# Dhia-naouali/dinov3-jax

Measured on NVIDIA H100. Metric: global_crops_per_sec, higher is better.
Workload: dtype bf16

## Files before the change

dinov3-jax_b200/csrc/gemm_tc.cu:

```cuda
#include <cstdlib>
#include <cstring>
#include "ptx.cuh"
#include "d3_internal.h"

namespace d3 {

constexpr int BM = 128;
constexpr int BK = 64;
constexpr int GEMM_THREADS = 384;

constexpr int EPI_RUNTIME = -1;
constexpr int EPI_FLAGS = EP_BIAS | EP_GELU | EP_STORE_PRE | EP_MUL_DGELU | EP_GAMMA | EP_RESID | EP_OUT_F32 | EP_ACCUM |
                          EP_SLABS;

template <int EF>
constexpr bool kStaged = EF != EPI_RUNTIME && (EF & (EP_SLABS | EP_ACCUM)) == 0;

template <int EF>
__device__ __forceinline__ bool epi_has(const GemmEpilogue& ep, int f) {
  return EF == EPI_RUNTIME ? (ep.flags & f) != 0 : (EF & f) != 0;
}

__device__ __forceinline__ float gelu_grad_epi(float u) {
  const float u2 = __fmul_rn(u, u);
// ... 15 lines not shown
  if (epi_has<EF>(ep, EP_ACCUM)) v = __fadd_rn(v, old);
  return v;
}

__device__ __forceinline__ float2 ld_pair(const float* p, bool vec, bool two) {
  if (vec) return *reinterpret_cast<const float2*>(p);
  return make_float2(p[0], two ? p[1] : 0.f);
}
__device__ __forceinline__ float2 ld_pair(const __nv_bfloat16* p, bool vec, bool two) {
  if (vec) return unpack_bf16(*reinterpret_cast<const uint32_t*>(p));
  return make_float2(__bfloat162float(p[0]), two ? __bfloat162float(p[1]) : 0.f);
}
__device__ __forceinline__ void st_pair(float* p, float a, float b, bool vec, bool two) {
  if (vec) {
    *reinterpret_cast<float2*>(p) = make_float2(a, b);
  } else {
    p[0] = a;
    if (two) p[1] = b;
  }
}
__device__ __forceinline__ void st_pair(__nv_bfloat16* p, float a, float b, bool vec, bool two) {
  if (vec) {
    *reinterpret_cast<uint32_t*>(p) = pack_bf16(a, b);
  } else {
    p[0] = __float2bfloat16(a);
    if (two) p[1] = __float2bfloat16(b);
  }
}

template <int BN>
__device__ __forceinline__ void epilogue_tile_runtime(const GemmEpilogue& ep, float (&acc)[2][BN / 2], int m0, int n0,
                                                      int M, int N, size_t slab_row0, int r_in, int c_in) {
  float* const out_f = reinterpret_cast<float*>(ep.out);
  __nv_bfloat16* const out_h = reinterpret_cast<__nv_bfloat16*>(ep.out);
  const bool aligned = (ep.flags & EP_SLOW) == 0;
#pragma unroll
  for (int mh = 0; mh < 2; ++mh)
#pragma unroll
    for (int h = 0; h < 2; ++h) {
      const size_t row = (size_t)(m0 + mh * 64 + r_in + 8 * h);
      if (row >= (size_t)M) continue;
      const size_t orow = slab_row0 + row;
#pragma unroll
      for (int i = 0; i < BN / 8; ++i) {
        const int n = n0 + 8 * i + c_in;
        if (n >= N) break;
        const bool two = n + 1 < N, vec = aligned && two;
        float2 b{}, u{}, g{}, x{}, o{};
        if (epi_has<EPI_RUNTIME>(ep, EP_BIAS)) b = ld_pair(ep.bias + n, vec, two);
        if (epi_has<EPI_RUNTIME>(ep, EP_MUL_DGELU)) u = ld_pair(ep.aux_in + row * ep.ld_aux + n, vec, two);
        if (epi_has<EPI_RUNTIME>(ep, EP_GAMMA)) g = ld_pair(ep.gamma + n, vec, two);
        if (epi_has<EPI_RUNTIME>(ep, EP_RESID)) x = ld_pair(ep.resid + row * ep.ld_resid + n, vec, two);
        if (epi_has<EPI_RUNTIME>(ep, EP_ACCUM)) o = ld_pair(out_f + orow * ep.ld_out + n, vec, two);
        float p0, p1;
        const float v0 = epi_value<EPI_RUNTIME>(ep, acc[mh][4 * i + 2 * h], b.x, u.x, g.x, x.x, o.x, p0);
        const float v1 = epi_value<EPI_RUNTIME>(ep, acc[mh][4 * i + 2 * h + 1], b.y, u.y, g.y, x.y, o.y, p1);
        if (epi_has<EPI_RUNTIME>(ep, EP_SCATTER)) {
          const unsigned long long g_idx = (unsigned long long)ep.sc_off + orow * ep.ld_out + n;
          const unsigned long long shard = (unsigned long long)ep.sc_shard;
          const unsigned r = (unsigned)(g_idx / shard);
          float* const dst = ep.sc_peer[r] + (g_idx - r * shard);
          if (!two) {
            atomicAdd(dst, v0);
          } else if (ep.sc_sys) {
            atomicAdd_system(dst, v0); atomicAdd_system(dst + 1, v1);
          } else {
            atomicAdd(reinterpret_cast<float2*>(dst), make_float2(v0, v1));
          }
          continue;
        }
        if (epi_has<EPI_RUNTIME>(ep, EP_STORE_PRE)) st_pair(ep.aux_out + row * ep.ld_aux + n, p0, p1, vec, two);
        if (epi_has<EPI_RUNTIME>(ep, EP_OUT_F32)) st_pair(out_f + orow * ep.ld_out + n, v0, v1, vec, two);
        else st_pair(out_h + orow * ep.ld_out + n, v0, v1, vec, two);
      }
    }
}

constexpr int STG_BOX = 64 * 128;
constexpr int STG_BYTES = 3 * STG_BOX;
__device__ __forceinline__ uint32_t sw128(int r, int byte) {
  return r * 128 + ((((byte >> 4) ^ r) & 7) << 4) + (byte & 15);
}

template <int BN, int EF>
__device__ __forceinline__ void epilogue_tile(const GemmEpilogue& ep, const CUtensorMap* tm_out,
                                              const CUtensorMap* tm_pre, float (&acc)[2][BN / 2], const float* s_bias,
                                              const float* s_gamma, uint8_t* stg, int& seq, int bar, int t, int m0,
                                              int n0, int M, int N, size_t slab_row0, int r_in, int c_in) {
  constexpr bool STAGED = kStaged<EF>;
  constexpr bool F32 = (EF & EP_OUT_F32) != 0;
  constexpr int OUT_BOXES = F32 ? 2 : 1;
  constexpr int CHUNK = (OUT_BOXES + ((EF & EP_STORE_PRE) ? 1 : 0)) * STG_BOX;
  constexpr int NBUF = STG_BYTES / CHUNK;
  static_assert(NBUF >= 1, "a chunk must fit the staging area");
  float* const out_f = reinterpret_cast<float*>(ep.out);
  __nv_bfloat16* const out_h = reinterpret_cast<__nv_bfloat16*>(ep.out);
#pragma unroll
  for (int mh = 0; mh < 2; ++mh)
#pragma unroll
    for (int cb = 0; cb < BN / 64; ++cb) {
      const int row0 = m0 + mh * 64, col0 = n0 + cb * 64;
      if (row0 >= M || col0 >= N) continue;
      float2 xr[2][8], xo[2][8];
      uint32_t xu[2][8];
#pragma unroll
      for (int h = 0; h < 2; ++h) {
        const size_t row = (size_t)row0 + r_in + 8 * h;
#pragma unroll
        for (int i = 0; i < 8; ++i) {
          const int n = col0 + 8 * i + c_in;
          if (row < (size_t)M && n < N) {
            if (epi_has<EF>(ep, EP_RESID))
              xr[h][i] = *reinterpret_cast<const float2*>(ep.resid + row * ep.ld_resid + n);
            if (epi_has<EF>(ep, EP_MUL_DGELU))
              xu[h][i] = *reinterpret_cast<const uint32_t*>(ep.aux_in + row * ep.ld_aux + n);
            if (epi_has<EF>(ep, EP_ACCUM))
              xo[h][i] = *reinterpret_cast<const float2*>(out_f + (slab_row0 + row) * ep.ld_out + n);
          }
        }
      }
      uint8_t* const buf = stg + (seq % NBUF) * CHUNK;
      if constexpr (STAGED) {
        if (t == 0) tma_store_wait_read<NBUF - 1>();
        named_bar_sync(bar, 128);
      }
#pragma unroll
      for (int h = 0; h < 2; ++h) {
        const int r = r_in + 8 * h;
        const size_t row = (size_t)row0 + r;
#pragma unroll
        for (int i = 0; i < 8; ++i) {
          const int cl = cb * 64 + 8 * i + c_in;
          const int n = n0 + cl;
          const float2 b = epi_has<EF>(ep, EP_BIAS) ? *reinterpret_cast<const float2*>(s_bias + cl) : float2{};
          const float2 g = epi_has<EF>(ep, EP_GAMMA) ? *reinterpret_cast<const float2*>(s_gamma + cl) : float2{};
          const float2 u = epi_has<EF>(ep, EP_MUL_DGELU) ? unpack_bf16(xu[h][i]) : float2{};
          float p0, p1;
          const float v0 = epi_value<EF>(ep, acc[mh][4 * (cl >> 3) + 2 * h], b.x, u.x, g.x, xr[h][i].x, xo[h][i].x, p0);
          const float v1 = epi_value<EF>(ep, acc[mh][4 * (cl >> 3) + 2 * h + 1], b.y, u.y, g.y, xr[h][i].y, xo[h][i].y,
                                         p1);
          if constexpr (STAGED) {
            if (epi_has<EF>(ep, EP_STORE_PRE))
              *reinterpret_cast<uint32_t*>(buf + OUT_BOXES * STG_BOX + sw128(r, 16 * i + 2 * c_in)) = pack_bf16(p0, p1);
            if constexpr (F32) {
              *reinterpret_cast<float2*>(buf + (i >> 2) * STG_BOX + sw128(r, 32 * (i & 3) + 4 * c_in)) =
                  make_float2(v0, v1);
            } else {
              *reinterpret_cast<uint32_t*>(buf + sw128(r, 16 * i + 2 * c_in)) = pack_bf16(v0, v1);
            }
          } else if (row < (size_t)M && n < N) {
            if (epi_has<EF>(ep, EP_STORE_PRE)) st_pair(ep.aux_out + row * ep.ld_aux + n, p0, p1, true, true);
            if constexpr (F32) st_pair(out_f + (slab_row0 + row) * ep.ld_out + n, v0, v1, true, true);
            else st_pair(out_h + (slab_row0 + row) * ep.ld_out + n, v0, v1, true, true);
          }
        }
      }
      if constexpr (STAGED) {
        fence_proxy_async_smem();
        named_bar_sync(bar, 128);
        if (t == 0) {
          tma_store_2d(tm_out, buf, col0, row0);
          if (F32 && col0 + 32 < N) tma_store_2d(tm_out, buf + STG_BOX, col0 + 32, row0);
          if constexpr ((EF & EP_STORE_PRE) != 0) tma_store_2d(tm_pre, buf + OUT_BOXES * STG_BOX, col0, row0);
          tma_store_commit();
        }
        ++seq;
      }
    }
}

template <int BN, bool STAGED>
struct Cfg {
  static constexpr int STAGES = (BN == 128 ? 6 : 8) - (STAGED ? 1 : 0);
  static constexpr int A_BYTES = BM * BK * 2;
  static constexpr int B_BYTES = BN * BK * 2;
  static constexpr int STAGE_BYTES = A_BYTES + B_BYTES;
  static constexpr int BAR_BYTES = 256;
  static constexpr int VEC_BYTES = 2 * 2 * BN * 4;
  static constexpr int VEC_END = STAGES * STAGE_BYTES + BAR_BYTES + VEC_BYTES;
  static constexpr int STG_OFF = (VEC_END + 1023) / 1024 * 1024;
  static constexpr int SMEM_BYTES = (STAGED ? STG_OFF + 2 * STG_BYTES : VEC_END) + 1024;
  static_assert(SMEM_BYTES <= 227 * 1024, "over the opt-in shared-memory limit");
};

struct WorkRange { int m0, n0, kb0, kb1; };
__device__ __forceinline__ WorkRange work_item(int w, int rank, int num_pairs, int num_k, int splits, int tile_n) {
  const int tile = w / splits, sp = w % splits;
  const int per = (num_k + splits - 1) / splits;
  WorkRange r;
  r.n0 = (2 * (tile % num_pairs) + rank) * tile_n;
  r.m0 = (tile / num_pairs) * BM;
  r.kb0 = sp * per;
  r.kb1 = min(num_k, r.kb0 + per);
  return r;
}

template <int BN, int A_MN, int B_MN>
__device__ __forceinline__ void mma_kblock(float (&acc)[2][BN / 2], uint32_t sa, uint32_t sb, bool first) {
  const uint64_t bd = B_MN ? gmma_desc_sw128(sb, 8192, 1024) : gmma_desc_sw128(sb, 16, 1024);
  constexpr uint64_t a_adv = A_MN ? (2048 >> 4) : (32 >> 4);
  constexpr uint64_t b_adv = B_MN ? (2048 >> 4) : (32 >> 4);
#pragma unroll
  for (int k = 0; k < BK / 16; ++k) {
    const uint32_t sc = (first && k == 0) ? 0u : 1u;
#pragma unroll
    for (int mh = 0; mh < 2; ++mh) {
      const uint64_t ad = A_MN ? gmma_desc_sw128(sa + mh * 8192, 8192, 1024) : gmma_desc_sw128(sa + mh * 8192, 16, 1024);
      if constexpr (BN == 128) wgmma_m64n128k16_ss<A_MN, B_MN>(acc[mh], ad + k * a_adv, bd + k * b_adv, sc);
      else wgmma_m64n64k16_ss<A_MN, B_MN>(acc[mh], ad + k * a_adv, bd + k * b_adv, sc);
    }
  }
}

template <int BN, int A_MN, int B_MN, int EF>
__global__ void __launch_bounds__(GEMM_THREADS, 1)
gemm_kernel(const __grid_constant__ CUtensorMap tmA, const __grid_constant__ CUtensorMap tmB,
            const __grid_constant__ CUtensorMap tmO, const __grid_constant__ CUtensorMap tmP, const GemmEpilogue ep,
            int M, int N, int K, int splits) {
  constexpr bool staged = kStaged<EF>;
  using C = Cfg<BN, staged>;
  static_assert(2 * C::STAGES * 8 <= C::BAR_BYTES, "mbarriers overflow their slot");
  extern __shared__ uint8_t smem_raw[];
  uint8_t* smem = reinterpret_cast<uint8_t*>((reinterpret_cast<uintptr_t>(smem_raw) + 1023) & ~uintptr_t(1023));
  uint64_t* full_bar = reinterpret_cast<uint64_t*>(smem + C::STAGES * C::STAGE_BYTES);
  uint64_t* empty_bar = full_bar + C::STAGES;
  float* vecs = reinterpret_cast<float*>(smem + C::STAGES * C::STAGE_BYTES + C::BAR_BYTES);

  const int wg = threadIdx.x >> 7;
  const int rank = blockIdx.x & 1;
  const int cluster = blockIdx.x >> 1, num_clusters = gridDim.x >> 1;
  if (threadIdx.x == 0) {
    tma_prefetch_desc(&tmA);
    tma_prefetch_desc(&tmB);
    if constexpr (staged) {
      tma_prefetch_desc(&tmO);
      if constexpr ((EF & EP_STORE_PRE) != 0) tma_prefetch_desc(&tmP);
    }
    for (int s = 0; s < C::STAGES; ++s) { mbar_init(&full_bar[s], 1); mbar_init(&empty_bar[s], 2); }
    fence_mbar_init();
  }
  cluster_sync();

  const int num_m = (M + BM - 1) / BM;
  const int num_pairs = ((N + BN - 1) / BN + 1) / 2;
  const int num_k = (K + BK - 1) / BK;
  const int num_work = num_m * num_pairs * splits;

  if (wg == 0) {
    setmaxnreg_dec<40>();
    if (threadIdx.x < 32 && elect_one()) {
      int stage = 0;
      uint32_t phase = 0;
      for (int w = cluster; w < num_work; w += num_clusters) {
        const WorkRange wr = work_item(w, rank, num_pairs, num_k, splits, BN);
        for (int kb = wr.kb0; kb < wr.kb1; ++kb) {
          mbar_wait(&empty_bar[stage], phase ^ 1);
          uint8_t* sa = smem + stage * C::STAGE_BYTES;
          uint8_t* sb = sa + C::A_BYTES;
          mbar_expect_tx(&full_bar[stage], C::STAGE_BYTES);
          if (A_MN) {
            tma_load_2d_multicast(&tmA, &full_bar[stage], sa + rank * 8192, wr.m0 + rank * 64, kb * BK, 0b11);
          } else {
            tma_load_2d_multicast(&tmA, &full_bar[stage], sa + rank * 8192, kb * BK, wr.m0 + rank * 64, 0b11);
          }
          if (B_MN) {
#pragma unroll
            for (int i = 0; i < BN / 64; ++i) tma_load_2d(&tmB, &full_bar[stage], sb + i * 8192, wr.n0 + i * 64, kb * BK);
          } else {
            tma_load_2d(&tmB, &full_bar[stage], sb, kb * BK, wr.n0);
          }
          if (++stage == C::STAGES) { stage = 0; phase ^= 1; }
        }
      }
    }
  } else {
    setmaxnreg_inc<232>();
    const int cw = wg - 1;
    const int t = threadIdx.x & 127;
    const int r_in = 16 * (t >> 5) + ((t & 31) >> 2);
    const int c_in = 2 * (t & 3);
    float* const s_bias = vecs + cw * 2 * BN;
    float* const s_gamma = s_bias + BN;
    constexpr bool stage_vecs = EF != EPI_RUNTIME && (EF & (EP_BIAS | EP_GAMMA)) != 0;
    uint8_t* const stg = smem + C::STG_OFF + cw * STG_BYTES;
    const uint32_t peer_empty = mapa_shared(smem_u32(empty_bar), rank ^ 1);
    int stg_seq = 0;
    int stage = 0;
    uint32_t phase = 0;
    int j = 0;
    for (int w = cluster; w < num_work; w += num_clusters, ++j) {
      const WorkRange wr = work_item(w, rank, num_pairs, num_k, splits, BN);
      const int nkb = wr.kb1 > wr.kb0 ? wr.kb1 - wr.kb0 : 0;
      if ((j & 1) != cw) {
        stage += nkb;
        phase ^= (stage / C::STAGES) & 1;
        stage %= C::STAGES;
        continue;
      }
      if constexpr (stage_vecs) {
        named_bar_sync(3 + cw, 128);
        if (t < BN && wr.n0 + t < N) {
          if constexpr ((EF & EP_BIAS) != 0) cp_async_4(s_bias + t, ep.bias + wr.n0 + t);
          if constexpr ((EF & EP_GAMMA) != 0) cp_async_4(s_gamma + t, ep.gamma + wr.n0 + t);
        }
      }
      if (j > 0) named_bar_sync(1 + cw, 256);
      float acc[2][BN / 2];
#pragma unroll
      for (int mh = 0; mh < 2; ++mh)
#pragma unroll
        for (int i = 0; i < BN / 2; ++i) acc[mh][i] = 0.f;
      int prev = -1;
      for (int kb = wr.kb0; kb < wr.kb1; ++kb) {
        mbar_wait(&full_bar[stage], phase);
        const uint32_t sa = smem_u32(smem + stage * C::STAGE_BYTES);
        fence_regs(acc[0]);
        fence_regs(acc[1]);
        wgmma_fence();
        mma_kblock<BN, A_MN, B_MN>(acc, sa, sa + C::A_BYTES, kb == wr.kb0);
        wgmma_commit();
        fence_regs(acc[0]);
        fence_regs(acc[1]);
        if (prev >= 0) {
          wgmma_wait<1>();
          if (t == 0) { mbar_arrive(&empty_bar[prev]); mbar_arrive_cluster(peer_empty + 8 * prev); }
        }
        prev = stage;
        if (++stage == C::STAGES) { stage = 0; phase ^= 1; }
      }
      if (w + num_clusters < num_work) named_bar_arrive(1 + (cw ^ 1), 256);
      wgmma_wait<0>();
      fence_regs(acc[0]);
      fence_regs(acc[1]);
      if (prev >= 0 && t == 0) { mbar_arrive(&empty_bar[prev]); mbar_arrive_cluster(peer_empty + 8 * prev); }
      if constexpr (stage_vecs) {
        cp_async_wait_all();
        named_bar_sync(3 + cw, 128);
      }
      if (nkb <= 0) continue;
      const size_t slab_row0 = epi_has<EF>(ep, EP_SLABS) ? (size_t)(w % splits) * M : 0;
      if constexpr (EF == EPI_RUNTIME) {
        epilogue_tile_runtime<BN>(ep, acc, wr.m0, wr.n0, M, N, slab_row0, r_in, c_in);
      } else {
        epilogue_tile<BN, EF>(ep, &tmO, &tmP, acc, s_bias, s_gamma, stg, stg_seq, 5 + cw, t, wr.m0, wr.n0, M, N,
                              slab_row0, r_in, c_in);
      }
    }
    if (staged && t == 0) tma_store_wait_all();
  }
  cluster_sync();
}

static int make_operand_map(CUtensorMap* map, const void* ptr, int mn, int k, int ld, int is_mn_major, int box_mn) {
  cuuint64_t dims[2], strides[1];
  cuuint32_t box[2], estr[2] = {1, 1};
  if (is_mn_major) {
    dims[0] = (cuuint64_t)mn; dims[1] = (cuuint64_t)k; box[0] = 64; box[1] = 64;
  } else {
    dims[0] = (cuuint64_t)k; dims[1] = (cuuint64_t)mn; box[0] = 64; box[1] = (cuuint32_t)box_mn;
  }
  strides[0] = (cuuint64_t)ld * 2;
  return encode_tensor_map_2d_bf16(map, ptr, dims, strides, box, estr);
}

template <int BN, int A_MN, int B_MN, int EF>
static int launch(const CUtensorMap& ta, const CUtensorMap& tb, const GemmEpilogue& ep, int M, int N, int K,
                  int splits, cudaStream_t stream) {
  using C = Cfg<BN, kStaged<EF>>;
  auto kern = gemm_kernel<BN, A_MN, B_MN, EF>;
  cudaLaunchAttribute attr{};
  attr.id = cudaLaunchAttributeClusterDimension;
  attr.val.clusterDim.x = 2;
  attr.val.clusterDim.y = 1;
  attr.val.clusterDim.z = 1;
  cudaLaunchConfig_t cfg{};
  cfg.blockDim = dim3(GEMM_THREADS);
  cfg.dynamicSmemBytes = C::SMEM_BYTES;
  cfg.stream = stream;
  cfg.attrs = &attr;
  cfg.numAttrs = 1;
  static int max_clusters = 0;
  if (max_clusters == 0) {
    cudaError_t e = cudaFuncSetAttribute(kern, cudaFuncAttributeMaxDynamicSharedMemorySize, C::SMEM_BYTES);
    if (e != cudaSuccess) return set_error(D3_ERR_CUDA, cudaGetErrorString(e));
    cfg.gridDim = dim3(2 * sm_count());
    e = cudaOccupancyMaxActiveClusters(&max_clusters, kern, &cfg);
    if (e != cudaSuccess) return set_error(D3_ERR_CUDA, cudaGetErrorString(e));
    if (max_clusters < 1) return set_error(D3_ERR_CUDA, "gemm: no 2-CTA cluster fits on the device");
  }
  CUtensorMap to{}, tp{};
  if constexpr (kStaged<EF>) {
    const int elt = (EF & EP_OUT_F32) ? 4 : 2;
    int rc = encode_tensor_map_2d(&to, ep.out, elt, N, M, (cuuint64_t)ep.ld_out * elt, 128 / elt, 64, 128);
    if (rc) return rc;
    if constexpr ((EF & EP_STORE_PRE) != 0) {
      rc = encode_tensor_map_2d(&tp, ep.aux_out, 2, N, M, (cuuint64_t)ep.ld_aux * 2, 64, 64, 128);
      if (rc) return rc;
    }
  }
  const int work = ((M + BM - 1) / BM) * (((N + BN - 1) / BN + 1) / 2) * splits;
  cfg.gridDim = dim3(2 * (work < max_clusters ? work : max_clusters));
  cudaError_t e = cudaLaunchKernelEx(&cfg, kern, ta, tb, to, tp, ep, M, N, K, splits);
  if (e == cudaSuccess) e = cudaPeekAtLastError();
  if (e != cudaSuccess) return set_error(D3_ERR_CUDA, cudaGetErrorString(e));
  count_launch();
  return D3_OK;
}

template <int BN>
static int dispatch(int a_mn, int b_mn, const CUtensorMap& ta, const CUtensorMap& tb, const GemmEpilogue& ep, int M,
                    int N, int K, int splits, cudaStream_t s) {
  if (!(ep.flags & (EP_SLOW | EP_SCATTER)) && N % 2 == 0) {
    const int f = ep.flags & EPI_FLAGS;
#define D3_EPI(A, B, F) \
    if (a_mn == A && b_mn == B && f == (F)) return launch<BN, A, B, (F)>(ta, tb, ep, M, N, K, splits, s);
    D3_EPI(0, 1, EP_BIAS)
    D3_EPI(0, 1, EP_BIAS | EP_OUT_F32)
    D3_EPI(0, 1, EP_BIAS | EP_GELU)
    D3_EPI(0, 1, EP_BIAS | EP_GELU | EP_STORE_PRE)
    D3_EPI(0, 1, EP_BIAS | EP_GAMMA | EP_RESID | EP_OUT_F32)
    D3_EPI(0, 1, EP_BIAS | EP_STORE_PRE | EP_GAMMA | EP_RESID | EP_OUT_F32)
    D3_EPI(0, 1, EP_BIAS | EP_GELU | EP_GAMMA | EP_RESID | EP_OUT_F32)
    D3_EPI(0, 1, EP_BIAS | EP_GELU | EP_STORE_PRE | EP_GAMMA | EP_RESID | EP_OUT_F32)
    D3_EPI(0, 1, EP_OUT_F32)
    D3_EPI(0, 0, 0)
    D3_EPI(0, 0, EP_MUL_DGELU)
    D3_EPI(0, 0, EP_OUT_F32)
    D3_EPI(1, 1, EP_OUT_F32 | EP_SLABS)
    D3_EPI(1, 1, EP_OUT_F32 | EP_ACCUM)
#undef D3_EPI
  }
  if (!a_mn && !b_mn) return launch<BN, 0, 0, EPI_RUNTIME>(ta, tb, ep, M, N, K, splits, s);
  if (!a_mn && b_mn) return launch<BN, 0, 1, EPI_RUNTIME>(ta, tb, ep, M, N, K, splits, s);
  if (a_mn && !b_mn) return launch<BN, 1, 0, EPI_RUNTIME>(ta, tb, ep, M, N, K, splits, s);
  return launch<BN, 1, 1, EPI_RUNTIME>(ta, tb, ep, M, N, K, splits, s);
}

int gemm_bf16(const void* A, int lda, int a_mn, const void* B, int ldb, int b_mn, int M, int N, int K,
              GemmEpilogue ep, int tile_n, int split_k, cudaStream_t stream) {
  if (M <= 0 || N <= 0 || K <= 0) return set_error(D3_ERR_ARG, "gemm: empty problem");
  if ((lda % 8) || (ldb % 8) || (reinterpret_cast<uintptr_t>(A) & 15) || (reinterpret_cast<uintptr_t>(B) & 15))
    return set_error(D3_ERR_ARG, "gemm: operands must be 16-byte aligned with ld % 8 == 0");
  const int sms = sm_count();
  const int num_k = (K + BK - 1) / BK;
  int bn = tile_n >= 256 ? 128 : tile_n;
  if (tile_n == 0) {
    const int cand[2] = {128, 64};
    long best = -1;
    for (int i = 0; i < 2; ++i) {
      const long tiles = (long)((M + BM - 1) / BM) * ((N + cand[i] - 1) / cand[i]);
      const long waves = (tiles + sms - 1) / sms;
      const long cost = waves * (cand[i] + 24);
      if (best < 0 || cost < best) { best = cost; bn = cand[i]; }
    }
  }
  const bool plain_f32 = (ep.flags & EP_OUT_F32) && !(ep.flags & (EP_BIAS | EP_GELU | EP_STORE_PRE | EP_MUL_DGELU |
                                                                  EP_GAMMA | EP_RESID));
  int splits = 1;
  if (split_k >= 1) {
    splits = split_k;
  } else if (plain_f32 && (ep.flags & EP_ACCUM)) {
    const long units = (long)((M + BM - 1) / BM) * ((N + bn - 1) / bn);
    if (units <= sms && num_k >= 16) {
      splits = units * 2 <= sms ? (int)(sms / units) : 1;
      if (splits < (num_k + 63) / 64) splits = (num_k + 63) / 64;
      if (splits > num_k / 4) splits = num_k / 4;
      if (splits < 1) splits = 1;
    }
  }
  if (ep.flags & EP_SCATTER) {
    if (!plain_f32) return set_error(D3_ERR_ARG, "gemm: SCATTER needs a plain fp32 output");
    if (ep.sc_world < 1 || ep.sc_world > 8 || ep.sc_shard <= 0 || (ep.sc_shard % 4) || (ep.sc_off % 4) || (ep.ld_out % 4))
      return set_error(D3_ERR_ARG, "gemm: SCATTER needs 1..8 ranks and 4-element aligned shard / offset / ld_out");
    if ((unsigned long long)ep.sc_off + (unsigned long long)(M - 1) * ep.ld_out + N > (unsigned long long)ep.sc_shard * ep.sc_world)
      return set_error(D3_ERR_ARG, "gemm: SCATTER output exceeds the sharded range");
  }
  if (splits > 1) {
    if (!plain_f32) return set_error(D3_ERR_ARG, "gemm: split-K needs a plain fp32 output");
    if (!(ep.flags & EP_ACCUM)) return set_error(D3_ERR_ARG, "gemm: split-K accumulates into out (set ACCUM, zero it first)");
    if (splits > num_k) splits = num_k;
  }
  if (ep.flags & EP_SCATTER) ep.flags &= ~EP_ACCUM;
  const int out_elt = (ep.flags & EP_OUT_F32) ? 4 : 2;
  bool aligned = ((uintptr_t)ep.out % 16 == 0) && ((ep.ld_out * out_elt) % 16 == 0);
  if (ep.flags & EP_BIAS) aligned = aligned && ((uintptr_t)ep.bias % 16 == 0);
  if (ep.flags & EP_GAMMA) aligned = aligned && ((uintptr_t)ep.gamma % 16 == 0);
  if (ep.flags & EP_RESID) aligned = aligned && ((uintptr_t)ep.resid % 16 == 0) && (ep.ld_resid % 4 == 0);
  if (ep.flags & EP_STORE_PRE) aligned = aligned && ((uintptr_t)ep.aux_out % 16 == 0) && (ep.ld_aux % 8 == 0);
  if (ep.flags & EP_MUL_DGELU) aligned = aligned && ((uintptr_t)ep.aux_in % 16 == 0) && (ep.ld_aux % 8 == 0);
  if (!aligned) ep.flags |= EP_SLOW;

  CUtensorMap ta, tb;
  int rc = make_operand_map(&ta, A, M, K, lda, a_mn, 64);
  if (rc) return rc;
  rc = make_operand_map(&tb, B, N, K, ldb, b_mn, bn);
  if (rc) return rc;
  float* ws = nullptr;
  GemmEpilogue out_ep = ep;
  if (splits > 1 && !(ep.flags & EP_SCATTER)) {
    ws = slab_workspace((size_t)splits * M * N, stream);
    if (!ws) return D3_ERR_CUDA;
    ep.out = ws;
    ep.ld_out = N;
    ep.flags = (ep.flags & ~(EP_ACCUM | EP_SLOW)) | EP_SLABS | (N % 4 ? EP_SLOW : 0);
  }
  switch (bn) {
    case 128: rc = dispatch<128>(a_mn, b_mn, ta, tb, ep, M, N, K, splits, stream); break;
    case 64: rc = dispatch<64>(a_mn, b_mn, ta, tb, ep, M, N, K, splits, stream); break;
    default: rc = set_error(D3_ERR_ARG, "gemm: bad tile N");
  }
  if (ws) {
    if (!rc) rc = slab_combine(ws, splits, (long long)M * N, M, N, reinterpret_cast<float*>(out_ep.out), out_ep.ld_out, stream);
    slab_release(ws, stream);
  }
  return rc;
}

}
```

dinov3-jax_b200/csrc/ptx.cuh:

```cuda
#pragma once
#include <cuda.h>
#include <cuda_runtime.h>
#include <cuda_bf16.h>
#include <stdint.h>

namespace d3 {

__device__ __forceinline__ uint32_t smem_u32(const void* p) {
  return static_cast<uint32_t>(__cvta_generic_to_shared(p));
}
__device__ __forceinline__ uint32_t lane_id() { return threadIdx.x & 31; }
__device__ __forceinline__ bool elect_one() {
  uint32_t pred;
  asm volatile("{\n\t.reg .pred p;\n\telect.sync _|p, 0xffffffff;\n\tselp.u32 %0, 1, 0, p;\n\t}" : "=r"(pred));
  return pred != 0;
}

__device__ __forceinline__ void mbar_init(uint64_t* bar, uint32_t count) {
  asm volatile("mbarrier.init.shared::cta.b64 [%0], %1;" ::"r"(smem_u32(bar)), "r"(count) : "memory");
}
__device__ __forceinline__ void fence_mbar_init() {
  asm volatile("fence.mbarrier_init.release.cluster;" ::: "memory");
}
__device__ __forceinline__ void mbar_expect_tx(uint64_t* bar, uint32_t bytes) {
// ... 39 lines not shown
  asm volatile("prefetch.tensormap [%0];" ::"l"(reinterpret_cast<uint64_t>(m)) : "memory");
}
__device__ __forceinline__ void tma_load_2d(const CUtensorMap* m, uint64_t* bar, void* dst, int c0, int c1) {
  asm volatile(
      "cp.async.bulk.tensor.2d.shared::cluster.global.mbarrier::complete_tx::bytes [%0], [%1, {%3, %4}], [%2];"
      ::"r"(smem_u32(dst)), "l"(reinterpret_cast<uint64_t>(m)), "r"(smem_u32(bar)), "r"(c0), "r"(c1)
      : "memory");
}
__device__ __forceinline__ void tma_load_2d_multicast(const CUtensorMap* m, uint64_t* bar, void* dst, int c0, int c1,
                                                      uint16_t cta_mask) {
  asm volatile(
      "cp.async.bulk.tensor.2d.shared::cluster.global.mbarrier::complete_tx::bytes.multicast::cluster"
      " [%0], [%1, {%3, %4}], [%2], %5;"
      ::"r"(smem_u32(dst)), "l"(reinterpret_cast<uint64_t>(m)), "r"(smem_u32(bar)), "r"(c0), "r"(c1), "h"(cta_mask)
      : "memory");
}

__device__ __forceinline__ uint32_t mapa_shared(uint32_t addr, uint32_t rank) {
  uint32_t r;
  asm volatile("mapa.shared::cluster.u32 %0, %1, %2;" : "=r"(r) : "r"(addr), "r"(rank));
  return r;
}
__device__ __forceinline__ void mbar_arrive_cluster(uint32_t cluster_addr) {
  asm volatile("mbarrier.arrive.shared::cluster.b64 _, [%0];" ::"r"(cluster_addr) : "memory");
}
__device__ __forceinline__ void cluster_sync() {
  asm volatile("barrier.cluster.arrive;\n\tbarrier.cluster.wait;" ::: "memory");
}

__device__ __forceinline__ void tma_store_2d(const CUtensorMap* m, const void* src, int c0, int c1) {
  asm volatile("cp.async.bulk.tensor.2d.global.shared::cta.bulk_group [%0, {%2, %3}], [%1];"
               ::"l"(reinterpret_cast<uint64_t>(m)), "r"(smem_u32(src)), "r"(c0), "r"(c1)
               : "memory");
}
__device__ __forceinline__ void tma_store_commit() { asm volatile("cp.async.bulk.commit_group;" ::: "memory"); }
template <int N>
__device__ __forceinline__ void tma_store_wait_read() { asm volatile("cp.async.bulk.wait_group.read %0;" ::"n"(N) : "memory"); }
__device__ __forceinline__ void tma_store_wait_all() { asm volatile("cp.async.bulk.wait_group 0;" ::: "memory"); }
__device__ __forceinline__ void tma_load_2d_cta(const CUtensorMap* m, uint64_t* bar, void* dst, int c0, int c1) {
  asm volatile(
      "cp.async.bulk.tensor.2d.shared::cta.global.mbarrier::complete_tx::bytes [%0], [%1, {%3, %4}], [%2];"
      ::"r"(smem_u32(dst)), "l"(reinterpret_cast<uint64_t>(m)), "r"(smem_u32(bar)), "r"(c0), "r"(c1)
      : "memory");
}

__device__ __forceinline__ uint64_t gmma_desc_sw128(uint32_t saddr, uint32_t lbo_bytes, uint32_t sbo_bytes) {
  uint64_t d = 0;
  d |= (uint64_t)((saddr >> 4) & 0x3FFF);
  d |= (uint64_t)((lbo_bytes >> 4) & 0x3FFF) << 16;
  d |= (uint64_t)((sbo_bytes >> 4) & 0x3FFF) << 32;
  d |= (uint64_t)1 << 62;
  return d;
}
__device__ __forceinline__ void wgmma_fence() { asm volatile("wgmma.fence.sync.aligned;" ::: "memory"); }
__device__ __forceinline__ void wgmma_commit() { asm volatile("wgmma.commit_group.sync.aligned;" ::: "memory"); }
template <int N>
__device__ __forceinline__ void wgmma_wait() { asm volatile("wgmma.wait_group.sync.aligned %0;" ::"n"(N) : "memory"); }
template <int R>
__device__ __forceinline__ void fence_regs(float (&d)[R]) {
#pragma unroll
  for (int i = 0; i < R; ++i) asm volatile("" : "+f"(d[i])::"memory");
}
template <int R>
__device__ __forceinline__ void setmaxnreg_inc() { asm volatile("setmaxnreg.inc.sync.aligned.u32 %0;" ::"n"(R)); }
template <int R>
__device__ __forceinline__ void setmaxnreg_dec() { asm volatile("setmaxnreg.dec.sync.aligned.u32 %0;" ::"n"(R)); }

template <int TA, int TB>
__device__ __forceinline__ void wgmma_m64n64k16_ss(float (&d)[32], uint64_t da, uint64_t db, uint32_t scale_d) {
  asm volatile(
      "{\n\t.reg .pred p;\n\tsetp.ne.b32 p, %34, 0;\n\t"
      "wgmma.mma_async.sync.aligned.m64n64k16.f32.bf16.bf16 {%0, %1, %2, %3, %4, %5, %6, %7, %8, %9, %10, %11, %12, %13, %14, %15, %16, %17, %18, %19, %20, %21, %22, %23, %24, %25, %26, %27, %28, %29, %30, %31}, %32, %33, p, 1, 1, %35, %36;\n\t}"
      : "+f"(d[0]), "+f"(d[1]), "+f"(d[2]), "+f"(d[3]), "+f"(d[4]), "+f"(d[5]), "+f"(d[6]), "+f"(d[7]), "+f"(d[8]), "+f"(d[9]), "+f"(d[10]), "+f"(d[11]), "+f"(d[12]), "+f"(d[13]), "+f"(d[14]), "+f"(d[15]), "+f"(d[16]), "+f"(d[17]), "+f"(d[18]), "+f"(d[19]), "+f"(d[20]), "+f"(d[21]), "+f"(d[22]), "+f"(d[23]), "+f"(d[24]), "+f"(d[25]), "+f"(d[26]), "+f"(d[27]), "+f"(d[28]), "+f"(d[29]), "+f"(d[30]), "+f"(d[31])
      : "l"(da), "l"(db), "r"(scale_d), "n"(TA), "n"(TB));
}
template <int TA, int TB>
__device__ __forceinline__ void wgmma_m64n128k16_ss(float (&d)[64], uint64_t da, uint64_t db, uint32_t scale_d) {
  asm volatile(
      "{\n\t.reg .pred p;\n\tsetp.ne.b32 p, %66, 0;\n\t"
      "wgmma.mma_async.sync.aligned.m64n128k16.f32.bf16.bf16 {%0, %1, %2, %3, %4, %5, %6, %7, %8, %9, %10, %11, %12, %13, %14, %15, %16, %17, %18, %19, %20, %21, %22, %23, %24, %25, %26, %27, %28, %29, %30, %31, %32, %33, %34, %35, %36, %37, %38, %39, %40, %41, %42, %43, %44, %45, %46, %47, %48, %49, %50, %51, %52, %53, %54, %55, %56, %57, %58, %59, %60, %61, %62, %63}, %64, %65, p, 1, 1, %67, %68;\n\t}"
      : "+f"(d[0]), "+f"(d[1]), "+f"(d[2]), "+f"(d[3]), "+f"(d[4]), "+f"(d[5]), "+f"(d[6]), "+f"(d[7]), "+f"(d[8]), "+f"(d[9]), "+f"(d[10]), "+f"(d[11]), "+f"(d[12]), "+f"(d[13]), "+f"(d[14]), "+f"(d[15]), "+f"(d[16]), "+f"(d[17]), "+f"(d[18]), "+f"(d[19]), "+f"(d[20]), "+f"(d[21]), "+f"(d[22]), "+f"(d[23]), "+f"(d[24]), "+f"(d[25]), "+f"(d[26]), "+f"(d[27]), "+f"(d[28]), "+f"(d[29]), "+f"(d[30]), "+f"(d[31]), "+f"(d[32]), "+f"(d[33]), "+f"(d[34]), "+f"(d[35]), "+f"(d[36]), "+f"(d[37]), "+f"(d[38]), "+f"(d[39]), "+f"(d[40]), "+f"(d[41]), "+f"(d[42]), "+f"(d[43]), "+f"(d[44]), "+f"(d[45]), "+f"(d[46]), "+f"(d[47]), "+f"(d[48]), "+f"(d[49]), "+f"(d[50]), "+f"(d[51]), "+f"(d[52]), "+f"(d[53]), "+f"(d[54]), "+f"(d[55]), "+f"(d[56]), "+f"(d[57]), "+f"(d[58]), "+f"(d[59]), "+f"(d[60]), "+f"(d[61]), "+f"(d[62]), "+f"(d[63])
      : "l"(da), "l"(db), "r"(scale_d), "n"(TA), "n"(TB));
}
template <int TB>
__device__ __forceinline__ void wgmma_m64n64k16_rs(float (&d)[32], const uint32_t (&a)[4], uint64_t db, uint32_t scale_d) {
  asm volatile(
      "{\n\t.reg .pred p;\n\tsetp.ne.b32 p, %37, 0;\n\t"
      "wgmma.mma_async.sync.aligned.m64n64k16.f32.bf16.bf16 {%0, %1, %2, %3, %4, %5, %6, %7, %8, %9, %10, %11, %12, %13, %14, %15, %16, %17, %18, %19, %20, %21, %22, %23, %24, %25, %26, %27, %28, %29, %30, %31}, {%32, %33, %34, %35}, %36, p, 1, 1, %38;\n\t}"
      : "+f"(d[0]), "+f"(d[1]), "+f"(d[2]), "+f"(d[3]), "+f"(d[4]), "+f"(d[5]), "+f"(d[6]), "+f"(d[7]), "+f"(d[8]), "+f"(d[9]), "+f"(d[10]), "+f"(d[11]), "+f"(d[12]), "+f"(d[13]), "+f"(d[14]), "+f"(d[15]), "+f"(d[16]), "+f"(d[17]), "+f"(d[18]), "+f"(d[19]), "+f"(d[20]), "+f"(d[21]), "+f"(d[22]), "+f"(d[23]), "+f"(d[24]), "+f"(d[25]), "+f"(d[26]), "+f"(d[27]), "+f"(d[28]), "+f"(d[29]), "+f"(d[30]), "+f"(d[31])
      : "r"(a[0]), "r"(a[1]), "r"(a[2]), "r"(a[3]), "l"(db), "r"(scale_d), "n"(TB));
}

__device__ __forceinline__ float ex2_approx(float x) {
  float y;
  asm("ex2.approx.ftz.f32 %0, %1;" : "=f"(y) : "f"(x));
  return y;
}
__device__ __forceinline__ float tanh_approx(float x) {
  float y;
  asm("tanh.approx.f32 %0, %1;" : "=f"(y) : "f"(x));
  return y;
}
__device__ __forceinline__ float gelu_tanh_fast(float u) {
  const float t = tanh_approx(u * (0.7978845608028654f + 0.0356774081363001f * u * u));
  const float h = 0.5f * u;
  return fmaf(h, t, h);
}
__device__ __forceinline__ float gelu_tanh_grad_fast(float u) {
  const float u2 = u * u;
  const float t = tanh_approx(u * (0.7978845608028654f + 0.0356774081363001f * u2));
  const float dz = 0.7978845608028654f + 0.1070322244089003f * u2;
  return 0.5f * (1.0f + t) + 0.5f * u * (1.0f - t * t) * dz;
}


__device__ __forceinline__ float gelu_tanh(float u) {
  float z = 0.7978845608028654f * (u + 0.044715f * u * u * u);
  float t = 1.0f - 2.0f / (__expf(2.0f * z) + 1.0f);
  return 0.5f * u * (1.0f + t);
}
__device__ __forceinline__ float gelu_tanh_grad(float u) {
  float u2 = u * u;
  float z = 0.7978845608028654f * (u + 0.044715f * u * u2);
  float t = 1.0f - 2.0f / (__expf(2.0f * z) + 1.0f);
  float dz = 0.7978845608028654f * (1.0f + 3.0f * 0.044715f * u2);
  return 0.5f * (1.0f + t) + 0.5f * u * (1.0f - t * t) * dz;
}
__device__ __forceinline__ uint32_t pack_bf16(float a, float b) {
  __nv_bfloat162 v = __floats2bfloat162_rn(a, b);
  return *reinterpret_cast<uint32_t*>(&v);
}
__device__ __forceinline__ float2 unpack_bf16(uint32_t u) {
  __nv_bfloat162 v = *reinterpret_cast<__nv_bfloat162*>(&u);
  return __bfloat1622float2(v);
}

}
```

Before: 370.4.

## Add 128x256 GEMM tile with cooperative consumer warpgroups and B multicast

Adds a BN=256 tile path in which both consumer warpgroups split one 128x256 tile, each issuing m64n256k16 wgmma on its own 64-row half. The cluster now pairs CTAs along M and multicasts the B operand, instead of pairing along N and multicasting A. When both operands are MN-major and no tile size is given, this wide tile is chosen by default. It aims to raise operand reuse and tensor-core efficiency per k-block, at the cost of fewer pipeline stages, higher register pressure from 128 fp32 accumulators per thread, and losing the ping-pong overlap of epilogue and MMA between warpgroups.

```diff
diff --git a/dinov3-jax_b200/csrc/gemm_tc.cu b/dinov3-jax_b200/csrc/gemm_tc.cu
--- a/dinov3-jax_b200/csrc/gemm_tc.cu
+++ b/dinov3-jax_b200/csrc/gemm_tc.cu
@@ -121,9 +121,9 @@
   return r * 128 + ((((byte >> 4) ^ r) & 7) << 4) + (byte & 15);
 }
 
-template <int BN, int EF>
+template <int MH, int BN, int EF>
 __device__ __forceinline__ void epilogue_tile(const GemmEpilogue& ep, const CUtensorMap* tm_out,
-                                              const CUtensorMap* tm_pre, float (&acc)[2][BN / 2], const float* s_bias,
+                                              const CUtensorMap* tm_pre, float (&acc)[MH][BN / 2], const float* s_bias,
                                               const float* s_gamma, uint8_t* stg, int& seq, int bar, int t, int m0,
                                               int n0, int M, int N, size_t slab_row0, int r_in, int c_in) {
   constexpr bool STAGED = kStaged<EF>;
@@ -135,7 +135,7 @@
   float* const out_f = reinterpret_cast<float*>(ep.out);
   __nv_bfloat16* const out_h = reinterpret_cast<__nv_bfloat16*>(ep.out);
 #pragma unroll
-  for (int mh = 0; mh < 2; ++mh)
+  for (int mh = 0; mh < MH; ++mh)
 #pragma unroll
     for (int cb = 0; cb < BN / 64; ++cb) {
       const int row0 = m0 + mh * 64, col0 = n0 + cb * 64;
@@ -210,32 +210,40 @@
 
 template <int BN, bool STAGED>
 struct Cfg {
-  static constexpr int STAGES = (BN == 128 ? 6 : 8) - (STAGED ? 1 : 0);
+  static constexpr bool WIDE = BN == 256;
+  static constexpr int STAGES = (BN == 256 ? 4 : BN == 128 ? 6 : 8) - (STAGED ? 1 : 0);
   static constexpr int A_BYTES = BM * BK * 2;
   static constexpr int B_BYTES = BN * BK * 2;
   static constexpr int STAGE_BYTES = A_BYTES + B_BYTES;
   static constexpr int BAR_BYTES = 256;
-  static constexpr int VEC_BYTES = 2 * 2 * BN * 4;
+  static constexpr int VEC_BYTES = (WIDE ? 1 : 2) * 2 * BN * 4;
   static constexpr int VEC_END = STAGES * STAGE_BYTES + BAR_BYTES + VEC_BYTES;
   static constexpr int STG_OFF = (VEC_END + 1023) / 1024 * 1024;
   static constexpr int SMEM_BYTES = (STAGED ? STG_OFF + 2 * STG_BYTES : VEC_END) + 1024;
   static_assert(SMEM_BYTES <= 227 * 1024, "over the opt-in shared-memory limit");
 };
 
-struct WorkRange { int m0, n0, kb0, kb1; };
-__device__ __forceinline__ WorkRange work_item(int w, int rank, int num_pairs, int num_k, int splits, int tile_n) {
-  const int tile = w / splits, sp = w % splits;
+struct WorkRange { int m0, n0, kb0, kb1, sp; };
+template <int BN>
+__device__ __forceinline__ WorkRange work_item(int w, int rank, int num_n, int num_tiles, int num_k, int splits) {
+  const int tile = w % num_tiles, sp = w / num_tiles;
   const int per = (num_k + splits - 1) / splits;
   WorkRange r;
-  r.n0 = (2 * (tile % num_pairs) + rank) * tile_n;
-  r.m0 = (tile / num_pairs) * BM;
+  if constexpr (BN == 256) {
+    r.n0 = (tile % num_n) * BN;
+    r.m0 = (2 * (tile / num_n) + rank) * BM;
+  } else {
+    r.n0 = (2 * (tile % num_n) + rank) * BN;
+    r.m0 = (tile / num_n) * BM;
+  }
   r.kb0 = sp * per;
   r.kb1 = min(num_k, r.kb0 + per);
+  r.sp = sp;
   return r;
 }
 
-template <int BN, int A_MN, int B_MN>
-__device__ __forceinline__ void mma_kblock(float (&acc)[2][BN / 2], uint32_t sa, uint32_t sb, bool first) {
+template <int MH, int BN, int A_MN, int B_MN>
+__device__ __forceinline__ void mma_kblock(float (&acc)[MH][BN / 2], uint32_t sa, uint32_t sb, bool first) {
   const uint64_t bd = B_MN ? gmma_desc_sw128(sb, 8192, 1024) : gmma_desc_sw128(sb, 16, 1024);
   constexpr uint64_t a_adv = A_MN ? (2048 >> 4) : (32 >> 4);
   constexpr uint64_t b_adv = B_MN ? (2048 >> 4) : (32 >> 4);
@@ -243,9 +251,10 @@
   for (int k = 0; k < BK / 16; ++k) {
     const uint32_t sc = (first && k == 0) ? 0u : 1u;
 #pragma unroll
-    for (int mh = 0; mh < 2; ++mh) {
+    for (int mh = 0; mh < MH; ++mh) {
       const uint64_t ad = A_MN ? gmma_desc_sw128(sa + mh * 8192, 8192, 1024) : gmma_desc_sw128(sa + mh * 8192, 16, 1024);
-      if constexpr (BN == 128) wgmma_m64n128k16_ss<A_MN, B_MN>(acc[mh], ad + k * a_adv, bd + k * b_adv, sc);
+      if constexpr (BN == 256) wgmma_m64n256k16_ss<A_MN, B_MN>(acc[mh], ad + k * a_adv, bd + k * b_adv, sc);
+      else if constexpr (BN == 128) wgmma_m64n128k16_ss<A_MN, B_MN>(acc[mh], ad + k * a_adv, bd + k * b_adv, sc);
       else wgmma_m64n64k16_ss<A_MN, B_MN>(acc[mh], ad + k * a_adv, bd + k * b_adv, sc);
     }
   }
@@ -258,6 +267,9 @@
             int M, int N, int K, int splits) {
   constexpr bool staged = kStaged<EF>;
   using C = Cfg<BN, staged>;
+  constexpr bool WIDE = C::WIDE;
+  constexpr int MH = WIDE ? 1 : 2;
+  static_assert(!WIDE || EF != EPI_RUNTIME, "run-time flags run on the 128-wide tile");
   static_assert(2 * C::STAGES * 8 <= C::BAR_BYTES, "mbarriers overflow their slot");
   extern __shared__ uint8_t smem_raw[];
   uint8_t* smem = reinterpret_cast<uint8_t*>((reinterpret_cast<uintptr_t>(smem_raw) + 1023) & ~uintptr_t(1023));
@@ -275,15 +287,16 @@
       tma_prefetch_desc(&tmO);
       if constexpr ((EF & EP_STORE_PRE) != 0) tma_prefetch_desc(&tmP);
     }
-    for (int s = 0; s < C::STAGES; ++s) { mbar_init(&full_bar[s], 1); mbar_init(&empty_bar[s], 2); }
+    for (int s = 0; s < C::STAGES; ++s) { mbar_init(&full_bar[s], 1); mbar_init(&empty_bar[s], WIDE ? 4 : 2); }
     fence_mbar_init();
   }
   cluster_sync();
 
   const int num_m = (M + BM - 1) / BM;
-  const int num_pairs = ((N + BN - 1) / BN + 1) / 2;
+  const int num_n = WIDE ? (N + BN - 1) / BN : ((N + BN - 1) / BN + 1) / 2;
   const int num_k = (K + BK - 1) / BK;
-  const int num_work = num_m * num_pairs * splits;
+  const int num_tiles = (WIDE ? (num_m + 1) / 2 : num_m) * num_n;
+  const int num_work = num_tiles * splits;
 
   if (wg == 0) {
     setmaxnreg_dec<40>();
@@ -291,22 +304,37 @@
       int stage = 0;
       uint32_t phase = 0;
       for (int w = cluster; w < num_work; w += num_clusters) {
-        const WorkRange wr = work_item(w, rank, num_pairs, num_k, splits, BN);
+        const WorkRange wr = work_item<BN>(w, rank, num_n, num_tiles, num_k, splits);
         for (int kb = wr.kb0; kb < wr.kb1; ++kb) {
           mbar_wait(&empty_bar[stage], phase ^ 1);
           uint8_t* sa = smem + stage * C::STAGE_BYTES;
           uint8_t* sb = sa + C::A_BYTES;
           mbar_expect_tx(&full_bar[stage], C::STAGE_BYTES);
-          if (A_MN) {
-            tma_load_2d_multicast(&tmA, &full_bar[stage], sa + rank * 8192, wr.m0 + rank * 64, kb * BK, 0b11);
+          if constexpr (WIDE) {
+#pragma unroll
+            for (int i = 0; i < 2; ++i) {
+              if (A_MN) tma_load_2d(&tmA, &full_bar[stage], sa + i * 8192, wr.m0 + i * 64, kb * BK);
+              else tma_load_2d(&tmA, &full_bar[stage], sa + i * 8192, kb * BK, wr.m0 + i * 64);
+            }
+            if (B_MN) {
+#pragma unroll
+              for (int i = 2 * rank; i < 2 * rank + 2; ++i)
+                tma_load_2d_multicast(&tmB, &full_bar[stage], sb + i * 8192, wr.n0 + i * 64, kb * BK, 0b11);
+            } else {
+              tma_load_2d_multicast(&tmB, &full_bar[stage], sb + rank * 16384, kb * BK, wr.n0 + rank * 128, 0b11);
+            }
           } else {
-            tma_load_2d_multicast(&tmA, &full_bar[stage], sa + rank * 8192, kb * BK, wr.m0 + rank * 64, 0b11);
-          }
-          if (B_MN) {
-#pragma unroll
-            for (int i = 0; i < BN / 64; ++i) tma_load_2d(&tmB, &full_bar[stage], sb + i * 8192, wr.n0 + i * 64, kb * BK);
-          } else {
-            tma_load_2d(&tmB, &full_bar[stage], sb, kb * BK, wr.n0);
+            if (A_MN) {
+              tma_load_2d_multicast(&tmA, &full_bar[stage], sa + rank * 8192, wr.m0 + rank * 64, kb * BK, 0b11);
+            } else {
+              tma_load_2d_multicast(&tmA, &full_bar[stage], sa + rank * 8192, kb * BK, wr.m0 + rank * 64, 0b11);
+            }
+            if (B_MN) {
+#pragma unroll
+              for (int i = 0; i < BN / 64; ++i) tma_load_2d(&tmB, &full_bar[stage], sb + i * 8192, wr.n0 + i * 64, kb * BK);
+            } else {
+              tma_load_2d(&tmB, &full_bar[stage], sb, kb * BK, wr.n0);
+            }
           }
           if (++stage == C::STAGES) { stage = 0; phase ^= 1; }
         }
@@ -318,9 +346,11 @@
     const int t = threadIdx.x & 127;
     const int r_in = 16 * (t >> 5) + ((t & 31) >> 2);
     const int c_in = 2 * (t & 3);
-    float* const s_bias = vecs + cw * 2 * BN;
+    float* const s_bias = vecs + (WIDE ? 0 : cw * 2 * BN);
     float* const s_gamma = s_bias + BN;
     constexpr bool stage_vecs = EF != EPI_RUNTIME && (EF & (EP_BIAS | EP_GAMMA)) != 0;
+    constexpr int VEC_THREADS = WIDE ? 256 : 128;
+    const int vt = WIDE ? threadIdx.x - 128 : t;
     uint8_t* const stg = smem + C::STG_OFF + cw * STG_BYTES;
     const uint32_t peer_empty = mapa_shared(smem_u32(empty_bar), rank ^ 1);
     int stg_seq = 0;
@@ -328,38 +358,38 @@
     uint32_t phase = 0;
     int j = 0;
     for (int w = cluster; w < num_work; w += num_clusters, ++j) {
-      const WorkRange wr = work_item(w, rank, num_pairs, num_k, splits, BN);
+      const WorkRange wr = work_item<BN>(w, rank, num_n, num_tiles, num_k, splits);
       const int nkb = wr.kb1 > wr.kb0 ? wr.kb1 - wr.kb0 : 0;
-      if ((j & 1) != cw) {
+      if (!WIDE && (j & 1) != cw) {
         stage += nkb;
         phase ^= (stage / C::STAGES) & 1;
         stage %= C::STAGES;
         continue;
       }
       if constexpr (stage_vecs) {
-        named_bar_sync(3 + cw, 128);
-        if (t < BN && wr.n0 + t < N) {
-          if constexpr ((EF & EP_BIAS) != 0) cp_async_4(s_bias + t, ep.bias + wr.n0 + t);
-          if constexpr ((EF & EP_GAMMA) != 0) cp_async_4(s_gamma + t, ep.gamma + wr.n0 + t);
-        }
-      }
-      if (j > 0) named_bar_sync(1 + cw, 256);
-      float acc[2][BN / 2];
-#pragma unroll
-      for (int mh = 0; mh < 2; ++mh)
+        named_bar_sync(3 + cw * !WIDE, VEC_THREADS);
+        if (vt < BN && wr.n0 + vt < N) {
+          if constexpr ((EF & EP_BIAS) != 0) cp_async_4(s_bias + vt, ep.bias + wr.n0 + vt);
+          if constexpr ((EF & EP_GAMMA) != 0) cp_async_4(s_gamma + vt, ep.gamma + wr.n0 + vt);
+        }
+      }
+      if (!WIDE && j > 0) named_bar_sync(1 + cw, 256);
+      float acc[MH][BN / 2];
+#pragma unroll
+      for (int mh = 0; mh < MH; ++mh)
 #pragma unroll
         for (int i = 0; i < BN / 2; ++i) acc[mh][i] = 0.f;
       int prev = -1;
       for (int kb = wr.kb0; kb < wr.kb1; ++kb) {
         mbar_wait(&full_bar[stage], phase);
         const uint32_t sa = smem_u32(smem + stage * C::STAGE_BYTES);
-        fence_regs(acc[0]);
-        fence_regs(acc[1]);
+#pragma unroll
+        for (int mh = 0; mh < MH; ++mh) fence_regs(acc[mh]);
         wgmma_fence();
-        mma_kblock<BN, A_MN, B_MN>(acc, sa, sa + C::A_BYTES, kb == wr.kb0);
+        mma_kblock<MH, BN, A_MN, B_MN>(acc, sa + (WIDE ? cw * 8192 : 0), sa + C::A_BYTES, kb == wr.kb0);
         wgmma_commit();
-        fence_regs(acc[0]);
-        fence_regs(acc[1]);
+#pragma unroll
+        for (int mh = 0; mh < MH; ++mh) fence_regs(acc[mh]);
         if (prev >= 0) {
           wgmma_wait<1>();
           if (t == 0) { mbar_arrive(&empty_bar[prev]); mbar_arrive_cluster(peer_empty + 8 * prev); }
@@ -367,22 +397,22 @@
         prev = stage;
         if (++stage == C::STAGES) { stage = 0; phase ^= 1; }
       }
-      if (w + num_clusters < num_work) named_bar_arrive(1 + (cw ^ 1), 256);
+      if (!WIDE && w + num_clusters < num_work) named_bar_arrive(1 + (cw ^ 1), 256);
       wgmma_wait<0>();
-      fence_regs(acc[0]);
-      fence_regs(acc[1]);
+#pragma unroll
+      for (int mh = 0; mh < MH; ++mh) fence_regs(acc[mh]);
       if (prev >= 0 && t == 0) { mbar_arrive(&empty_bar[prev]); mbar_arrive_cluster(peer_empty + 8 * prev); }
       if constexpr (stage_vecs) {
         cp_async_wait_all();
-        named_bar_sync(3 + cw, 128);
+        named_bar_sync(3 + cw * !WIDE, VEC_THREADS);
       }
       if (nkb <= 0) continue;
-      const size_t slab_row0 = epi_has<EF>(ep, EP_SLABS) ? (size_t)(w % splits) * M : 0;
+      const size_t slab_row0 = epi_has<EF>(ep, EP_SLABS) ? (size_t)wr.sp * M : 0;
       if constexpr (EF == EPI_RUNTIME) {
         epilogue_tile_runtime<BN>(ep, acc, wr.m0, wr.n0, M, N, slab_row0, r_in, c_in);
       } else {
-        epilogue_tile<BN, EF>(ep, &tmO, &tmP, acc, s_bias, s_gamma, stg, stg_seq, 5 + cw, t, wr.m0, wr.n0, M, N,
-                              slab_row0, r_in, c_in);
+        epilogue_tile<MH, BN, EF>(ep, &tmO, &tmP, acc, s_bias, s_gamma, stg, stg_seq, 5 + cw, t,
+                                  wr.m0 + (WIDE ? cw * 64 : 0), wr.n0, M, N, slab_row0, r_in, c_in);
       }
     }
     if (staged && t == 0) tma_store_wait_all();
@@ -437,7 +467,8 @@
       if (rc) return rc;
     }
   }
-  const int work = ((M + BM - 1) / BM) * (((N + BN - 1) / BN + 1) / 2) * splits;
+  const int num_m = (M + BM - 1) / BM, num_n = (N + BN - 1) / BN;
+  const int work = (BN == 256 ? (num_m + 1) / 2 * num_n : num_m * ((num_n + 1) / 2)) * splits;
   cfg.gridDim = dim3(2 * (work < max_clusters ? work : max_clusters));
   cudaError_t e = cudaLaunchKernelEx(&cfg, kern, ta, tb, to, tp, ep, M, N, K, splits);
   if (e == cudaSuccess) e = cudaPeekAtLastError();
@@ -469,10 +500,14 @@
     D3_EPI(1, 1, EP_OUT_F32 | EP_ACCUM)
 #undef D3_EPI
   }
-  if (!a_mn && !b_mn) return launch<BN, 0, 0, EPI_RUNTIME>(ta, tb, ep, M, N, K, splits, s);
-  if (!a_mn && b_mn) return launch<BN, 0, 1, EPI_RUNTIME>(ta, tb, ep, M, N, K, splits, s);
-  if (a_mn && !b_mn) return launch<BN, 1, 0, EPI_RUNTIME>(ta, tb, ep, M, N, K, splits, s);
-  return launch<BN, 1, 1, EPI_RUNTIME>(ta, tb, ep, M, N, K, splits, s);
+  if constexpr (BN == 256) {
+    return dispatch<128>(a_mn, b_mn, ta, tb, ep, M, N, K, splits, s);
+  } else {
+    if (!a_mn && !b_mn) return launch<BN, 0, 0, EPI_RUNTIME>(ta, tb, ep, M, N, K, splits, s);
+    if (!a_mn && b_mn) return launch<BN, 0, 1, EPI_RUNTIME>(ta, tb, ep, M, N, K, splits, s);
+    if (a_mn && !b_mn) return launch<BN, 1, 0, EPI_RUNTIME>(ta, tb, ep, M, N, K, splits, s);
+    return launch<BN, 1, 1, EPI_RUNTIME>(ta, tb, ep, M, N, K, splits, s);
+  }
 }
 
 int gemm_bf16(const void* A, int lda, int a_mn, const void* B, int ldb, int b_mn, int M, int N, int K,
@@ -482,7 +517,7 @@
     return set_error(D3_ERR_ARG, "gemm: operands must be 16-byte aligned with ld % 8 == 0");
   const int sms = sm_count();
   const int num_k = (K + BK - 1) / BK;
-  int bn = tile_n >= 256 ? 128 : tile_n;
+  int bn = tile_n >= 256 ? 256 : tile_n;
   if (tile_n == 0) {
     const int cand[2] = {128, 64};
     long best = -1;
@@ -499,7 +534,8 @@
   if (split_k >= 1) {
     splits = split_k;
   } else if (plain_f32 && (ep.flags & EP_ACCUM)) {
-    const long units = (long)((M + BM - 1) / BM) * ((N + bn - 1) / bn);
+    const int unit_n = bn < 128 ? bn : 128;
+    const long units = (long)((M + BM - 1) / BM) * ((N + unit_n - 1) / unit_n);
     if (units <= sms && num_k >= 16) {
       splits = units * 2 <= sms ? (int)(sms / units) : 1;
       if (splits < (num_k + 63) / 64) splits = (num_k + 63) / 64;
@@ -507,6 +543,7 @@
       if (splits < 1) splits = 1;
     }
   }
+  if (tile_n == 0 && a_mn && b_mn) bn = 256;
   if (ep.flags & EP_SCATTER) {
     if (!plain_f32) return set_error(D3_ERR_ARG, "gemm: SCATTER needs a plain fp32 output");
     if (ep.sc_world < 1 || ep.sc_world > 8 || ep.sc_shard <= 0 || (ep.sc_shard % 4) || (ep.sc_off % 4) || (ep.ld_out % 4))
@@ -532,7 +569,7 @@
   CUtensorMap ta, tb;
   int rc = make_operand_map(&ta, A, M, K, lda, a_mn, 64);
   if (rc) return rc;
-  rc = make_operand_map(&tb, B, N, K, ldb, b_mn, bn);
+  rc = make_operand_map(&tb, B, N, K, ldb, b_mn, bn < 128 ? bn : 128);
   if (rc) return rc;
   float* ws = nullptr;
   GemmEpilogue out_ep = ep;
@@ -544,6 +581,7 @@
     ep.flags = (ep.flags & ~(EP_ACCUM | EP_SLOW)) | EP_SLABS | (N % 4 ? EP_SLOW : 0);
   }
   switch (bn) {
+    case 256: rc = dispatch<256>(a_mn, b_mn, ta, tb, ep, M, N, K, splits, stream); break;
     case 128: rc = dispatch<128>(a_mn, b_mn, ta, tb, ep, M, N, K, splits, stream); break;
     case 64: rc = dispatch<64>(a_mn, b_mn, ta, tb, ep, M, N, K, splits, stream); break;
     default: rc = set_error(D3_ERR_ARG, "gemm: bad tile N");
diff --git a/dinov3-jax_b200/csrc/ptx.cuh b/dinov3-jax_b200/csrc/ptx.cuh
--- a/dinov3-jax_b200/csrc/ptx.cuh
+++ b/dinov3-jax_b200/csrc/ptx.cuh
@@ -145,6 +145,14 @@
       : "+f"(d[0]), "+f"(d[1]), "+f"(d[2]), "+f"(d[3]), "+f"(d[4]), "+f"(d[5]), "+f"(d[6]), "+f"(d[7]), "+f"(d[8]), "+f"(d[9]), "+f"(d[10]), "+f"(d[11]), "+f"(d[12]), "+f"(d[13]), "+f"(d[14]), "+f"(d[15]), "+f"(d[16]), "+f"(d[17]), "+f"(d[18]), "+f"(d[19]), "+f"(d[20]), "+f"(d[21]), "+f"(d[22]), "+f"(d[23]), "+f"(d[24]), "+f"(d[25]), "+f"(d[26]), "+f"(d[27]), "+f"(d[28]), "+f"(d[29]), "+f"(d[30]), "+f"(d[31]), "+f"(d[32]), "+f"(d[33]), "+f"(d[34]), "+f"(d[35]), "+f"(d[36]), "+f"(d[37]), "+f"(d[38]), "+f"(d[39]), "+f"(d[40]), "+f"(d[41]), "+f"(d[42]), "+f"(d[43]), "+f"(d[44]), "+f"(d[45]), "+f"(d[46]), "+f"(d[47]), "+f"(d[48]), "+f"(d[49]), "+f"(d[50]), "+f"(d[51]), "+f"(d[52]), "+f"(d[53]), "+f"(d[54]), "+f"(d[55]), "+f"(d[56]), "+f"(d[57]), "+f"(d[58]), "+f"(d[59]), "+f"(d[60]), "+f"(d[61]), "+f"(d[62]), "+f"(d[63])
       : "l"(da), "l"(db), "r"(scale_d), "n"(TA), "n"(TB));
 }
+template <int TA, int TB>
+__device__ __forceinline__ void wgmma_m64n256k16_ss(float (&d)[128], uint64_t da, uint64_t db, uint32_t scale_d) {
+  asm volatile(
+      "{\n\t.reg .pred p;\n\tsetp.ne.b32 p, %130, 0;\n\t"
+      "wgmma.mma_async.sync.aligned.m64n256k16.f32.bf16.bf16 {%0, %1, %2, %3, %4, %5, %6, %7, %8, %9, %10, %11, %12, %13, %14, %15, %16, %17, %18, %19, %20, %21, %22, %23, %24, %25, %26, %27, %28, %29, %30, %31, %32, %33, %34, %35, %36, %37, %38, %39, %40, %41, %42, %43, %44, %45, %46, %47, %48, %49, %50, %51, %52, %53, %54, %55, %56, %57, %58, %59, %60, %61, %62, %63, %64, %65, %66, %67, %68, %69, %70, %71, %72, %73, %74, %75, %76, %77, %78, %79, %80, %81, %82, %83, %84, %85, %86, %87, %88, %89, %90, %91, %92, %93, %94, %95, %96, %97, %98, %99, %100, %101, %102, %103, %104, %105, %106, %107, %108, %109, %110, %111, %112, %113, %114, %115, %116, %117, %118, %119, %120, %121, %122, %123, %124, %125, %126, %127}, %128, %129, p, 1, 1, %131, %132;\n\t}"
+      : "+f"(d[0]), "+f"(d[1]), "+f"(d[2]), "+f"(d[3]), "+f"(d[4]), "+f"(d[5]), "+f"(d[6]), "+f"(d[7]), "+f"(d[8]), "+f"(d[9]), "+f"(d[10]), "+f"(d[11]), "+f"(d[12]), "+f"(d[13]), "+f"(d[14]), "+f"(d[15]), "+f"(d[16]), "+f"(d[17]), "+f"(d[18]), "+f"(d[19]), "+f"(d[20]), "+f"(d[21]), "+f"(d[22]), "+f"(d[23]), "+f"(d[24]), "+f"(d[25]), "+f"(d[26]), "+f"(d[27]), "+f"(d[28]), "+f"(d[29]), "+f"(d[30]), "+f"(d[31]), "+f"(d[32]), "+f"(d[33]), "+f"(d[34]), "+f"(d[35]), "+f"(d[36]), "+f"(d[37]), "+f"(d[38]), "+f"(d[39]), "+f"(d[40]), "+f"(d[41]), "+f"(d[42]), "+f"(d[43]), "+f"(d[44]), "+f"(d[45]), "+f"(d[46]), "+f"(d[47]), "+f"(d[48]), "+f"(d[49]), "+f"(d[50]), "+f"(d[51]), "+f"(d[52]), "+f"(d[53]), "+f"(d[54]), "+f"(d[55]), "+f"(d[56]), "+f"(d[57]), "+f"(d[58]), "+f"(d[59]), "+f"(d[60]), "+f"(d[61]), "+f"(d[62]), "+f"(d[63]), "+f"(d[64]), "+f"(d[65]), "+f"(d[66]), "+f"(d[67]), "+f"(d[68]), "+f"(d[69]), "+f"(d[70]), "+f"(d[71]), "+f"(d[72]), "+f"(d[73]), "+f"(d[74]), "+f"(d[75]), "+f"(d[76]), "+f"(d[77]), "+f"(d[78]), "+f"(d[79]), "+f"(d[80]), "+f"(d[81]), "+f"(d[82]), "+f"(d[83]), "+f"(d[84]), "+f"(d[85]), "+f"(d[86]), "+f"(d[87]), "+f"(d[88]), "+f"(d[89]), "+f"(d[90]), "+f"(d[91]), "+f"(d[92]), "+f"(d[93]), "+f"(d[94]), "+f"(d[95]), "+f"(d[96]), "+f"(d[97]), "+f"(d[98]), "+f"(d[99]), "+f"(d[100]), "+f"(d[101]), "+f"(d[102]), "+f"(d[103]), "+f"(d[104]), "+f"(d[105]), "+f"(d[106]), "+f"(d[107]), "+f"(d[108]), "+f"(d[109]), "+f"(d[110]), "+f"(d[111]), "+f"(d[112]), "+f"(d[113]), "+f"(d[114]), "+f"(d[115]), "+f"(d[116]), "+f"(d[117]), "+f"(d[118]), "+f"(d[119]), "+f"(d[120]), "+f"(d[121]), "+f"(d[122]), "+f"(d[123]), "+f"(d[124]), "+f"(d[125]), "+f"(d[126]), "+f"(d[127])
+      : "l"(da), "l"(db), "r"(scale_d), "n"(TA), "n"(TB));
+}
 template <int TB>
 __device__ __forceinline__ void wgmma_m64n64k16_rs(float (&d)[32], const uint32_t (&a)[4], uint64_t db, uint32_t scale_d) {
   asm volatile(
```

After: 411.5 (median of 6 runs). 11.1% higher.
